# uzh-rpg/RVT

Hardware: AMD Instinct MI355X
Metric: event-tensors/sec (fwd+bwd) RVT-Base T=21 1Mpx; % MFMA roofline (higher is better)
Workload: dtype bf16; 1 GPU; RVT-Base, 1Mpx 20x360x640 (padded 384x640), T=21, B=24/GPU; global_batch=24, seq_len=21, parallelism=dp1, optimizer=AdamW(fused), hipgraph=off, upstream_grads=random cotangents on stage 2-4 features of all T frames

## Files before the change

### rvt_amd/csrc/attn_block.hpp

```cpp
#pragma once
#include "common.hpp"
#include "attn_pieces.hpp"
#include "opm.hpp"
#include "acc_frags.hpp"
#include "ln_pieces.hpp"

namespace rvt {

template <class T, int C> struct AbSmem {
    static constexpr int KT = C / TileGeom<T>::BK;
    static constexpr int W_QKV = KT * 3 * C * 128;
    static constexpr int W_P = KT * C * 128;
    static constexpr int OFF_P = W_QKV, OFF_K = W_QKV + W_P;
    static constexpr int K_LNW = 0, K_LNB = C, K_BQKV = 2 * C, K_BP = 5 * C, K_GAM = 6 * C, NCONST = 7 * C;
    static constexpr int OFF_S = OFF_K + NCONST * 4;
};

template <class T, int C>
__device__ __forceinline__ void ab_proj_t(f32x16& acc, const char* Wl, int wrows, int row0, const frag_t<T> (&uf)[C / 16], int li, int half) {
#pragma unroll
    for (int ks = 0; ks < C / 16; ks++) mma32(acc, opm_load_frag<T>(Wl, wrows, row0 + li, 2 * ks + half), uf[ks]);
}
template <class T, int C>
__device__ __forceinline__ void ab_proj_n(f32x16& acc, const char* Wl, int wrows, int row0, const frag_t<T> (&uf)[C / 16], int li, int half) {
// ... 358 lines not shown
#pragma unroll
            for (int bj = 0; bj < NB; bj++) {
                emit_dqkv(dk[bj], bj, r0 + 32);
                emit_dqkv(dv[bj], bj, r0 + 64);
            }
        }

#pragma unroll
        for (int b = 0; b < NB; b++) {
            float d8[KS][8];
#pragma unroll
            for (int cb = 0; cb < NCB; cb++) {
                float r8[2][8];
                acc_to_rows(du[cb][b], r8);
#pragma unroll
                for (int m = 0; m < 2; m++)
#pragma unroll
                    for (int e = 0; e < 8; e++) d8[2 * cb + m][e] = pt.valid[b] ? r8[m][e] : 0.f;
            }
            if (LN || PRE) {
                float gsum = 0.f, gxsum = 0.f;
                float xh[KS][8];
                if (PRE) {
#pragma unroll
                    for (int ks = 0; ks < KS; ks++)
#pragma unroll
                        for (int e = 0; e < 8; e++) d8[ks][e] += (float)df[b][ks][e];
                }
#pragma unroll
                for (int ks = 0; ks < KS; ks++) {
                    float w[8];
                    load_cols<8>(kst + S::K_LNW, 16 * ks + 8 * half, w);
                    const frag_t<T> xr = STASH ? *reinterpret_cast<const frag_t<T>*>(stash + (b * KS + ks) * 1024)
                                               : frag_load<T>((PRE ? y0 : x) + (size_t)pt.tok[b] * C + (2 * ks + half) * 8);
#pragma unroll
                    for (int e = 0; e < 8; e++) {
                        xh[ks][e] = pt.valid[b] ? ((float)xr[e] - mean[b]) * rstd[b] : 0.f;
                        const float gw = d8[ks][e] * w[e];
                        gsum += gw;
                        gxsum += gw * xh[ks][e];
                    }
                }
#pragma unroll
                for (int cb = 0; cb < NCB; cb++) {
                    f32x16 tw, tb;
                    acc_zero(tw);
                    acc_zero(tb);
#pragma unroll
                    for (int m = 0; m < 2; m++) {
                        float pw[8];
#pragma unroll
                        for (int e = 0; e < 8; e++) pw[e] = d8[2 * cb + m][e] * xh[2 * cb + m][e];
                        mma32(tw, frag_from_float<T>(pw), idf[m]);
                        mma32(tb, frag_from_float<T>(d8[2 * cb + m]), idf[m]);
                    }
#pragma unroll
                    for (int r = 0; r < 16; r++) { aw[cb] += tw[r]; ab[cb] += tb[r]; }
                }
                gsum += __shfl_xor(gsum, 32);
                gxsum += __shfl_xor(gxsum, 32);
                const float m1 = gsum / (float)C, m2 = gxsum / (float)C;
#pragma unroll
                for (int ks = 0; ks < KS; ks++) {
                    float w[8], o[8];
                    load_cols<8>(kst + S::K_LNW, 16 * ks + 8 * half, w);
#pragma unroll
                    for (int e = 0; e < 8; e++)
                        o[e] = (PRE ? 0.f : (float)df[b][ks][e]) + rstd[b] * (d8[ks][e] * w[e] - m1 - xh[ks][e] * m2);
                    if (pt.valid[b]) frag_store<T>(dx + (size_t)pt.tok[b] * C + (2 * ks + half) * 8, frag_from_float<T>(o));
                }
            } else {
#pragma unroll
                for (int ks = 0; ks < KS; ks++) {
                    float o[8];
#pragma unroll
                    for (int e = 0; e < 8; e++) o[e] = (float)df[b][ks][e] + d8[ks][e];
                    if (pt.valid[b]) frag_store<T>(dx + (size_t)pt.tok[b] * C + (2 * ks + half) * 8, frag_from_float<T>(o));
                }
            }
        }
    }
    if (LN || PRE) {
        float* const red = reinterpret_cast<float*>(smem + S::OFF_S + WPB * (SC::BYTES + DLN));
#pragma unroll
        for (int cb = 0; cb < NCB; cb++) {
            const float a = aw[cb] + __shfl_xor(aw[cb], 32), b = ab[cb] + __shfl_xor(ab[cb], 32);
            if (half == 0) {
                red[wave * 2 * C + 32 * cb + li] = a;
                red[wave * 2 * C + C + 32 * cb + li] = b;
            }
        }
        __syncthreads();
        for (int v = tid; v < 2 * C; v += 64 * WPB) {
            float sum = 0.f;
            for (int w = 0; w < WPB; w++) sum += red[w * 2 * C + v];
            atomicAdd((v < C ? dln_w : dln_b) + (v % C), sum);
        }
    }
}

}
```

### rvt_amd/csrc/mlp_chain.hpp

```cpp
#pragma once
#include "common.hpp"
#include "opm.hpp"
#include "acc_frags.hpp"
#include "ln_pieces.hpp"
#include "gelu_lut.hpp"

namespace rvt {

template <class T, int C> struct McSmem {
    static constexpr int KT = C / TileGeom<T>::BK, HID = 4 * C;
    static constexpr int W_1 = KT * HID * 128;
    static constexpr int W_2 = (HID / TileGeom<T>::BK) * C * 128;
    static constexpr int K_LNW = 0, K_LNB = C, K_B2 = 2 * C, K_GAM = 3 * C, K_B1 = 4 * C, NCONST = 8 * C;
};

template <class T, int C, int WPB, int MINW>
__global__ void __launch_bounds__(64 * WPB, MINW)
mlpc_fwd_kernel(const T* __restrict__ xmid, T* __restrict__ xout, const float* __restrict__ ln_w, const float* __restrict__ ln_b,
                const T* __restrict__ W1, const float* __restrict__ b1, const T* __restrict__ W2, const float* __restrict__ b2,
                const float* __restrict__ gamma, int M, float eps) {
    typedef McSmem<T, C> S;
    constexpr int KS = C / 16, NCB = C / 32, HID = 4 * C, NJC = HID / 32;
    __shared__ __attribute__((aligned(16))) char smem[S::W_1 + S::W_2 + S::NCONST * 4 + GeluTab<T>::BYTES];
    char* const W1_l = smem;
// ... 343 lines not shown
        }
        bf16x4 o;
#pragma unroll
        for (int r = 0; r < 4; r++) o[r] = (T)(acc[r] + acc2[r]);
        *reinterpret_cast<bf16x4*>(PB + buf * (32 * MCW_PP) + (16 * tb + l15) * MCW_PP + (16 * cq + 4 * kg) * 2) = o;
    };
    auto lnbwd = [&](const Stage& st, int buf, int tile, int slot) {
        if (!DGRAD || tile < 0 || tile >= n_tiles) return;
        const int row = tile * 32 + srow;
        const bf16x4 xb = __builtin_bit_cast(bf16x4, st.x), db = __builtin_bit_cast(bf16x4, st.d);
        const bf16x4 gb = *reinterpret_cast<const bf16x4*>(PB + buf * (32 * MCW_PP) + srow * MCW_PP + spc * 8);
        const float mean = MR[((slot & 3) * 32 + srow) * 2], rstd = MR[((slot & 3) * 32 + srow) * 2 + 1];
        float x[4];
#pragma unroll
        for (int i = 0; i < 4; i++) x[i] = (float)xb[i] - mean;
        float gw[4], s1 = 0.f, s2x = 0.f;
#pragma unroll
        for (int i = 0; i < 4; i++) {
            const float g = (float)gb[i];
            x[i] *= rstd;
            gw[i] = g * lw[i];
            s1 += gw[i];
            s2x += gw[i] * x[i];
            aw[i] += g * x[i];
            ab[i] += g;
        }
        const float m1 = row16_sum(s1) * (1.0f / C), m2 = row16_sum(s2x) * (1.0f / C);
        bf16x4 o;
#pragma unroll
        for (int i = 0; i < 4; i++) o[i] = (T)((float)db[i] + rstd * (gw[i] - m1 - x[i] * m2));
        if (row < M) *reinterpret_cast<bf16x4*>(dxmid + (size_t)row * C + 4 * spc) = o;
    };
    const bool mfma_first = wave < 4;
    const int t0 = blockIdx.x, G = gridDim.x;
    Stage sa, sb, sla, slb;
    fetch(sa, t0);
    fetch(sb, t0 + G);
    __syncthreads();
    stash(sa, t0, 0, 0);
    fetch(sa, t0 + 2 * G);
    if (DGRAD) fetch(sla, -1);
    lds_barrier();
    int k = 0;
    int tile = t0;
    for (; tile < n_tiles; tile += 2 * G, k += 2) {
        if (mfma_first) compute(0);
        stash(sb, tile + G, 1, k + 1);
        fetch(sb, tile + 3 * G);
        if (DGRAD) fetch(slb, tile - G);
        if (!mfma_first) compute(0);
        duty(1, tile - G, k - 1);
        lnbwd(sla, 0, tile - 2 * G, k - 2);
        lds_barrier();
        if (mfma_first && tile + G < n_tiles) compute(1);
        stash(sa, tile + 2 * G, 0, k + 2);
        fetch(sa, tile + 4 * G);
        if (DGRAD) fetch(sla, tile);
        if (!mfma_first && tile + G < n_tiles) compute(1);
        duty(0, tile, k);
        lnbwd(slb, 1, tile - G, k - 1);
        lds_barrier();
    }
    if (DGRAD) {
        fetch(slb, tile - G);
        duty(1, tile - G, k - 1);
        lnbwd(sla, 0, tile - 2 * G, k - 2);
        lds_barrier();
        lnbwd(slb, 1, tile - G, k - 1);
    }
    const size_t nwg = gridDim.x, wg = blockIdx.x;
    float* const p_dw1 = ws + wg * (size_t)(HID * C);
    float* const p_s2 = ws + nwg * (size_t)(HID * C) + wg * (size_t)(C * HID);
    float* const p_db1 = ws + 2 * nwg * (size_t)(HID * C) + (wg * 2) * (size_t)HID;
    float* const p_cs2 = ws + 2 * nwg * (size_t)(HID * C) + 2 * nwg * (size_t)HID + wg * (size_t)C;
#pragma unroll
    for (int cb = 0; cb < NCB; cb++)
#pragma unroll
        for (int r = 0; r < 16; r++) {
            p_dw1[(size_t)(32 * wave + acc_row(r, lane)) * C + 32 * cb + li] = dw1[cb][r];
            p_s2[(size_t)(32 * cb + acc_row(r, lane)) * HID + 32 * wave + li] = s2[cb][r];
        }
    db1 += __shfl_xor(db1, 32);
    if (half == 0) {
        p_db1[32 * wave + li] = db1;
        p_db1[HID + 32 * wave + li] = 0.f;
    }
    float* const red = reinterpret_cast<float*>(smem);
    __syncthreads();
#pragma unroll
    for (int i = 0; i < 4; i++) red[srow * C + 4 * spc + i] = cs[i];
    __syncthreads();
    if (tid < C) {
        float s = 0.f;
        for (int r = 0; r < 32; r++) s += red[r * C + tid];
        p_cs2[tid] = s;
    }
    if (DGRAD) {
        __syncthreads();
#pragma unroll
        for (int i = 0; i < 4; i++) { red[srow * C + 4 * spc + i] = aw[i]; red[32 * C + srow * C + 4 * spc + i] = ab[i]; }
        __syncthreads();
        if (tid < 2 * C) {
            float s = 0.f;
            for (int r = 0; r < 32; r++) s += red[(tid / C) * 32 * C + r * C + (tid % C)];
            atomicAdd((tid < C ? dln_w : dln_b) + (tid % C), s);
        }
    }
}

}
```

### rvt_amd/csrc/mlp_stream.hpp

```cpp
#pragma once
#include "common.hpp"
#include "lds_dma.hpp"
#include "opm.hpp"
#include "acc_frags.hpp"
#include "ln_pieces.hpp"
#include "gelu_lut.hpp"

namespace rvt {

template <class T, int C, int HC_ = TileGeom<T>::BK> struct MsGeom {
    static constexpr int BK = TileGeom<T>::BK;
    static constexpr int HC = HC_;
    static constexpr int KT = C / BK;
    static constexpr int HID = 4 * C, NCH = HID / HC, JPC = HC / 32;
    static constexpr int W1C = KT * HC * 128;
    static constexpr int W2C = C * 128;
    static constexpr int STAGE = W1C + W2C;
    static constexpr int K_LNW = 0, K_LNB = C, K_B2 = 2 * C, K_GAM = 3 * C, K_B1 = 4 * C, NCONST = 8 * C;
};

__device__ __forceinline__ int ms_rowperm(int li) { return (li & ~12) | ((li & 4) << 1) | ((li & 8) >> 1); }

template <class T, int C, int WPB, int MINW, int ABL = 0>
__global__ void __launch_bounds__(64 * WPB, MINW)
// ... 151 lines not shown
#pragma unroll
                for (int e = 0; e < 8; e++) o[e] = rs[e] + gam[e] * (r8[m][e] + b2v[e]);
                orow[ks] = frag_from_float<T>(o);
            }
        }
        prow = row;
        pvalid = valid;
    }
    if (pvalid) {
        const int half = lane_ >> 5;
#pragma unroll
        for (int ks = 0; ks < KS; ks++) frag_store<T>(xout + (size_t)prow * C + (2 * ks + half) * 8, orow[ks]);
    }
}



template <class T> struct MsTrAddr {
    int lo[2], hi[2];
    __device__ __forceinline__ void init(int lane, const char* smem) {
        const int rl = 4 * (lane >> 5) + ((lane & 15) >> 2), cl = 16 * ((lane >> 4) & 1) + 4 * (lane & 3);
        const int byte = cl * (int)sizeof(T);
#ifdef RVT_EMU
        const int base = 0;
        (void)smem;
#else
        const int base = (int)(size_t)(__attribute__((address_space(3))) const char*)(smem);
#endif
        const int l = rl * 128 + ((((byte >> 4) & 7) ^ ms_swz(rl)) << 4) + (byte & 15);
        const int h = (rl + 8) * 128 + ((((byte >> 4) & 7) ^ ms_swz(rl + 8)) << 4) + (byte & 15);
        lo[0] = base + l; lo[1] = base + (l ^ 64);
        hi[0] = base + h; hi[1] = base + (h ^ 64);
    }
};
#ifndef RVT_EMU
__device__ __forceinline__ void ms_lgkm_wait() {
    asm volatile("s_waitcnt lgkmcnt(0)" ::: "memory");
    __builtin_amdgcn_sched_barrier(0);
}
#else
__device__ __forceinline__ void ms_lgkm_wait() {}
#endif
template <int IMG, int ROWS, int ROW0, int CB>
__device__ __forceinline__ bf16x8 ms_tr_frag(const char* smem, const MsTrAddr<bf16>& a) {
    constexpr int OFF = IMG + (CB / 2) * ROWS * 128 + ROW0 * 128;
#ifdef RVT_EMU
    return frag_from_tr<bf16>(reinterpret_cast<const bf16*>(smem + OFF + a.lo[CB & 1]), reinterpret_cast<const bf16*>(smem + OFF + a.hi[CB & 1]));
#else
    typedef __attribute__((ext_vector_type(2))) unsigned int u32x2_t;
    u32x2_t lo, hi2;
    asm volatile("ds_read_b64_tr_b16 %0, %1 offset:%2" : "=v"(lo) : "v"(a.lo[CB & 1]), "n"(OFF));
    asm volatile("ds_read_b64_tr_b16 %0, %1 offset:%2" : "=v"(hi2) : "v"(a.hi[CB & 1]), "n"(OFF));
    const u32x4 v = {lo[0], lo[1], hi2[0], hi2[1]};
    bf16x8 f;
    __builtin_memcpy(&f, &v, 16);
    return f;
#endif
}
template <int ROWS>
__device__ __forceinline__ f32x8 ms_tr_frag_f32(const char* img, int row0, int col0, int lane) {
    f32x8 f;
#pragma unroll
    for (int e = 0; e < 8; e++) {
        const int row = row0 + (e & 3) + 8 * (e >> 2) + 4 * (lane >> 5), col = col0 + (lane & 31);
        const int byte = (col % 32) * 4;
        f[e] = *reinterpret_cast<const float*>(img + (col / 32) * ROWS * 128 + row * 128 + ((((byte >> 4) & 7) ^ ms_swz(row)) << 4) + (byte & 15));
    }
    return f;
}

template <class T, int C, int WPB, int MINW>
__global__ void __launch_bounds__(64 * WPB, MINW)
mlps_bwd_dgrad_kernel(const T* __restrict__ dxout, const T* __restrict__ xmid, T* __restrict__ dxmid,
                      const float* __restrict__ ln_w, const float* __restrict__ ln_b, const T* __restrict__ W1,
                      const float* __restrict__ b1, const T* __restrict__ W2gT, float* __restrict__ dln_w,
                      float* __restrict__ dln_b, int M, float eps) {
    typedef MsGeom<T, C, 32> G;
    constexpr int KS = C / 16, NCB = C / 32, HID = 4 * C, NCH = G::NCH, JPC = G::JPC;
    constexpr int NPW = (G::W1C / 1024) / WPB;
    static_assert(NPW * WPB * 1024 == G::W1C, "chunk pieces must divide over the waves");
    constexpr int STAGE = 2 * G::W1C;
    constexpr int DT = G::KT * 32 * 128;
    constexpr int OFF_DT = 2 * STAGE, OFF_K = OFF_DT + WPB * DT, OFF_LUT = OFF_K + G::NCONST * 4, OFF_PF = OFF_LUT + GeluTab<T>::BYTES;
    __shared__ __attribute__((aligned(16))) char smem[OFF_PF + 1024];
    float* const kst = reinterpret_cast<float*>(smem + OFF_K);
    float* const lut = reinterpret_cast<float*>(smem + OFF_LUT);
    const int tid = threadIdx.x, lane_ = tid & 63;
    const int wave = wave_uniform(tid >> 6);
    GeluTab<T>::template fill<true>(lut, tid, 64 * WPB);
    for (int i = tid; i < C; i += 64 * WPB) { kst[G::K_LNW + i] = ln_w[i]; kst[G::K_LNB + i] = ln_b[i]; }
    for (int i = tid; i < HID; i += 64 * WPB) kst[G::K_B1 + i] = b1[i];
    __syncthreads();

    const pp_rsrc r1 = pp_make_rsrc(W1, (unsigned)(HID * C * sizeof(T))), r2 = pp_make_rsrc(W2gT, (unsigned)(HID * C * sizeof(T)));
    auto issue = [&](int ch, int stage) __attribute__((always_inline)) {
        int lane = lane_;
        opaque_vgpr(lane);
        int v[NPW];
        ms_piece_offsets<T, NPW, WPB>(v, wave, lane, G::HC, C);
#pragma unroll
        for (int i = 0; i < NPW; i++) {
            const int p = wave + i * WPB;
            pp_glds16(r1, smem, stage * STAGE + p * 1024, v[i], ch * (G::HC * C * (int)sizeof(T)));
            pp_glds16(r2, smem, stage * STAGE + G::W1C + p * 1024, v[i], ch * (G::HC * C * (int)sizeof(T)));
        }
    };

    float aw[NCB], ab[NCB];
#pragma unroll
    for (int cb = 0; cb < NCB; cb++) { aw[cb] = 0.f; ab[cb] = 0.f; }

    const int n_tiles = (M + 31) / 32;
    const int n_wg = (n_tiles + WPB - 1) / WPB;
    char* const pf_dummy = smem + OFF_PF;
    issue(0, 0);
    frag_t<T> orow[KS];
    int prow = 0;
    bool pvalid = false;
    for (int twg = blockIdx.x; twg < n_wg; twg += gridDim.x) {
        int lane = lane_;
        opaque_vgpr(lane);
        const int li = lane & 31, half = lane >> 5;
        const int rb = ms_rowbase_h<T>(li, half);
        const int rbd = OFF_DT + wave * DT + rb;
        MsTrAddr<T> ta;
        ta.init(lane, smem);
        const int tile = twg * WPB + wave;
        const int row = tile * 32 + li;
        const bool valid = tile < n_tiles && row < M;
        const bool more = twg + (int)gridDim.x < n_wg;
        frag_t<T> uf[KS];
        float mean, rstd;
        {
            frag_t<T> xf[KS], df[KS];
            mc_load_row<T, C>(xf, xmid, row, valid, half);
            mc_load_row<T, C>(df, dxout, row, valid, half);
#pragma unroll
            for (int ks = 0; ks < KS; ks++) ms_store_frag<T>(smem, 32, rbd, 2 * ks, df[ks]);
            mc_layernorm<T, C>(xf, uf, kst + G::K_LNW, kst + G::K_LNB, valid, half, eps, mean, rstd);
        }
        f32x16 dacc[NCB];
#pragma unroll
        for (int cb = 0; cb < NCB; cb++) acc_zero(dacc[cb]);
        auto boundary = [&](int ch, int stage_next) __attribute__((always_inline)) {
            pp_wait_vm<0>();
            pp_barrier();
            if (ch + 1 < NCH) issue(ch + 1, stage_next);
            else if (more) issue(0, stage_next);
        };
        auto compute = [&](int ch, auto stage_c) __attribute__((always_inline)) {
            constexpr int STG = decltype(stage_c)::value;
            const char* const W1s = smem + STG * STAGE;
            const char* const W2s = W1s + G::W1C;
#pragma unroll
            for (int jj = 0; jj < JPC; jj++) {
                f32x16 h, dg;
                acc_load_rows(h, kst + G::K_B1 + ch * G::HC + 32 * jj, half);
                acc_zero(dg);
#pragma unroll
                for (int ks = 0; ks < KS; ks++) {
                    mma32(h, ms_load_frag<T>(W1s + 32 * jj * 128, G::HC, rb, 2 * ks), uf[ks]);
                    mma32(dg, ms_load_frag<T>(W2s + 32 * jj * 128, G::HC, rb, 2 * ks), ms_load_frag<T>(smem, 32, rbd, 2 * ks));
                }
                sched_fence();
                frag_t<T> wt[NCB][2];
                static_for<JPC>([&](auto jj_c) {
                    if (decltype(jj_c)::value != jj) return;
                    static_for<NCB * 2>([&](auto i_c) {
                        constexpr int JJ = decltype(jj_c)::value, CB = decltype(i_c)::value / 2, Q = decltype(i_c)::value % 2;
                        if constexpr (sizeof(T) == 2) wt[CB][Q] = ms_tr_frag<STG * STAGE, G::HC, 32 * JJ + 16 * Q, CB>(smem, ta);
                        else wt[CB][Q] = ms_tr_frag_f32<G::HC>(W1s, 32 * JJ + 16 * Q, CB * 32, lane);
                    });
                });
                float dh[16];
                GeluTab<T>::eval16(lut, h, dh);
#pragma unroll
                for (int r = 0; r < 16; r++) dh[r] = mul_nopack(dh[r], dg[r], r);
                frag_t<T> dhf[2];
                dhf[0] = arr_slot_frag<T>(dh, 0);
                dhf[1] = arr_slot_frag<T>(dh, 1);
                if constexpr (sizeof(T) == 2) ms_lgkm_wait();
#pragma unroll
                for (int cb = 0; cb < NCB; cb++)
#pragma unroll
                    for (int q = 0; q < 2; q++) mma32(dacc[cb], wt[cb][q], dhf[q]);
            }
        };
        boundary(0, 1);
        if (pvalid) {
#pragma unroll
            for (int ks = 0; ks < KS; ks++) frag_store<T>(dxmid + (size_t)prow * C + (2 * ks + half) * 8, orow[ks]);
        }
        compute(0, std::integral_constant<int, 0>());
#pragma unroll 1
        for (int ch = 1; ch < NCH - 1; ch += 2) {
            boundary(ch, 0);
            if (ch == 1 && more) {
                const int tn = tile + (int)gridDim.x * WPB;
                if (tn < n_tiles) {
                    const int rows = M - tn * 32 < 32 ? M - tn * 32 : 32;
                    const pp_rsrc rx = pp_make_rsrc(xmid + (size_t)tn * 32 * C, (unsigned)(rows * C * sizeof(T)));
                    const pp_rsrc rd = pp_make_rsrc(dxout + (size_t)tn * 32 * C, (unsigned)(rows * C * sizeof(T)));
#pragma unroll
                    for (int i = 0; i < (32 * C * (int)sizeof(T)) / 1024; i++) {
                        pp_glds16(rx, smem, (int)(pf_dummy - smem), lane * 16 + i * 1024, 0);
                        pp_glds16(rd, smem, (int)(pf_dummy - smem), lane * 16 + i * 1024, 0);
                    }
                }
            }
            compute(ch, std::integral_constant<int, 1>());
            boundary(ch + 1, 1);
            compute(ch + 1, std::integral_constant<int, 0>());
        }
        boundary(NCH - 1, 0);
        compute(NCH - 1, std::integral_constant<int, 1>());
        sched_fence();
        frag_t<T> xf[KS];
#pragma unroll
        for (int ks = 0; ks < KS; ks++) xf[ks] = frag_load<T>(xmid + (size_t)(valid ? row : 0) * C + (2 * ks + half) * 8);
        frag_t<T> idf[2];
#pragma unroll
        for (int m = 0; m < 2; m++)
#pragma unroll
            for (int e = 0; e < 8; e++) idf[m][e] = (T)((16 * m + 8 * half + e == li) ? 1.0f : 0.0f);
        float gsum = 0.f, gxsum = 0.f;
#pragma unroll
        for (int cb = 0; cb < NCB; cb++) {
            float r8[2][8];
            acc_to_rows(dacc[cb], r8);
            f32x16 tw, tb;
            acc_zero(tw);
            acc_zero(tb);
#pragma unroll
            for (int m = 0; m < 2; m++) {
                const int ks = 2 * cb + m;
                float w[8], pw[8], d[8];
                load_cols<8>(kst + G::K_LNW, 16 * ks + 8 * half, w);
#pragma unroll
                for (int e = 0; e < 8; e++) {
                    d[e] = valid ? r8[m][e] : 0.f;
                    const float xh = valid ? ((float)xf[ks][e] - mean) * rstd : 0.f;
                    const float gw = d[e] * w[e];
                    gsum += gw;
                    gxsum += gw * xh;
                    pw[e] = d[e] * xh;
                }
                mma32(tw, frag_from_float<T>(pw), idf[m]);
                mma32(tb, frag_from_float<T>(d), idf[m]);
            }
#pragma unroll
            for (int r = 0; r < 16; r++) { aw[cb] += tw[r]; ab[cb] += tb[r]; }
        }
        gsum += __shfl_xor(gsum, 32);
        gxsum += __shfl_xor(gxsum, 32);
        const float m1 = gsum / (float)C, m2 = gxsum / (float)C;
#pragma unroll
        for (int cb = 0; cb < NCB; cb++) {
            float r8[2][8];
#ifndef RVT_EMU
            asm volatile("" : "+v"(dacc[cb]));
#endif
            acc_to_rows(dacc[cb], r8);
#pragma unroll
            for (int m = 0; m < 2; m++) {
                const int ks = 2 * cb + m;
                float w[8], o[8];
                load_cols<8>(kst + G::K_LNW, 16 * ks + 8 * half, w);
                const frag_t<T> dfk = ms_load_frag<T>(smem, 32, rbd, 2 * ks);
#pragma unroll
                for (int e = 0; e < 8; e++) {
                    const float xh = ((float)xf[ks][e] - mean) * rstd;
                    o[e] = (float)dfk[e] + rstd * (r8[m][e] * w[e] - m1 - xh * m2);
                }
                orow[ks] = frag_from_float<T>(o);
            }
        }
        prow = row;
        pvalid = valid;
    }
    const int li = lane_ & 31, half = lane_ >> 5;
    if (pvalid) {
#pragma unroll
        for (int ks = 0; ks < KS; ks++) frag_store<T>(dxmid + (size_t)prow * C + (2 * ks + half) * 8, orow[ks]);
    }
    pp_wait_vm<0>();
    __syncthreads();
    float* const red = reinterpret_cast<float*>(smem);
#pragma unroll
    for (int cb = 0; cb < NCB; cb++) {
        const float a = aw[cb] + __shfl_xor(aw[cb], 32), b = ab[cb] + __shfl_xor(ab[cb], 32);
        if (half == 0) {
            red[wave * 2 * C + 32 * cb + li] = a;
            red[wave * 2 * C + C + 32 * cb + li] = b;
        }
    }
    __syncthreads();
    for (int v = tid; v < 2 * C; v += 64 * WPB) {
        float sum = 0.f;
        for (int w = 0; w < WPB; w++) sum += red[w * 2 * C + v];
        atomicAdd((v < C ? dln_w : dln_b) + (v % C), sum);
    }
}

struct MswGeom {
    static constexpr int C = 128, HID = 512, HB = 256, KS = 8, NCB = 4;
    static constexpr int TILE = 32 * 256;
    static constexpr int W2P = 272, W2IMG = HB * W2P;
    static constexpr int OFF_XV = 0, OFF_DX = 3 * TILE, OFF_W2 = 6 * TILE, OFF_LUT = OFF_W2 + W2IMG, OFF_K = OFF_LUT + GELU_NLUT_BYTES;
    static constexpr int SMEM = OFF_K + 2 * C * 4;
};
__device__ __forceinline__ int msw_tile_off(int row, int chunk) { return row * 256 + ((chunk ^ (row & 15)) << 4); }

template <int TAG>
__global__ void __launch_bounds__(512, 2)
mlps_bwd_wgrad_kernel(const bf16* __restrict__ dxout, const bf16* __restrict__ xmid, const float* __restrict__ ln_w,
                      const float* __restrict__ ln_b, const bf16* __restrict__ W1, const float* __restrict__ b1,
                      const bf16* __restrict__ W2gT, float* __restrict__ ws, int M, float eps, int nstreams) {
    typedef bf16 T;
    typedef MswGeom G;
    constexpr int C = G::C, KS = G::KS, NCB = G::NCB, HID = G::HID, TILE = G::TILE;
    __shared__ __attribute__((aligned(16))) char smem[G::SMEM];
    float* const lut = reinterpret_cast<float*>(smem + G::OFF_LUT);
    float* const kst = reinterpret_cast<float*>(smem + G::OFF_K);
    const int tid = threadIdx.x, lane_ = tid & 63;
    const int wave = wave_uniform(tid >> 6);
    const int bid = blockIdx.x;
    const int hb = (bid >> 3) & 1, stream = (bid >> 4) * 8 + (bid & 7);
    if (stream >= nstreams) return;
    const int n_tiles = (M + 31) / 32;
    const int count = stream < n_tiles ? (n_tiles - stream + nstreams - 1) / nstreams : 0;

    gelu_nlut_fill<false>(lut, tid, 512);
    for (int i = tid; i < C; i += 512) { kst[i] = ln_w[i]; kst[C + i] = ln_b[i]; }
    for (int f = tid; f < G::HB * 16; f += 512) {
        const int r = f >> 4, c = f & 15;
        *reinterpret_cast<u32x4*>(smem + G::OFF_W2 + r * G::W2P + c * 16) =
            *reinterpret_cast<const u32x4*>(W2gT + (size_t)(hb * G::HB + r) * C + c * 8);
    }
    const int jrow = hb * G::HB + 32 * wave + (lane_ & 31);
    frag_t<T> w1f[KS];
#pragma unroll
    for (int ks = 0; ks < KS; ks++) w1f[ks] = frag_load<T>(W1 + (size_t)jrow * C + 16 * ks + 8 * (lane_ >> 5));
    const float b1v = b1[jrow];

    f32x16 dw1[NCB], s2[NCB];
#pragma unroll
    for (int cb = 0; cb < NCB; cb++) { acc_zero(dw1[cb]); acc_zero(s2[cb]); }
    float db1 = 0.f;
    float cs1 = 0.f;
    const int cs_cb = wave & 3, cs_q = wave >> 2;

    auto issue = [&](int k, int buf) __attribute__((always_inline)) {
        int lane = lane_;
        opaque_vgpr(lane);
        const int tile = stream + k * nstreams;
        const int rows = tile < n_tiles ? (M - tile * 32 < 32 ? M - tile * 32 : 32) : 0;
        const pp_rsrc rx = pp_make_rsrc(xmid + (size_t)(rows ? tile : 0) * 32 * C, (unsigned)(rows * C * 2));
        const pp_rsrc rd = pp_make_rsrc(dxout + (size_t)(rows ? tile : 0) * 32 * C, (unsigned)(rows * C * 2));
        const int r = 4 * wave + (lane >> 4), c = (lane & 15) ^ (r & 15);
        const int voff = r * 256 + c * 16;
        pp_glds16(rx, smem, G::OFF_XV + buf * TILE + wave * 1024, voff, 0);
        pp_glds16(rd, smem, G::OFF_DX + buf * TILE + wave * 1024, voff, 0);
    };
    auto layernorm = [&](int buf, bool live) __attribute__((always_inline)) {
        if (!live) return;
        int t = tid;
        opaque_vgpr(t);
        const int srow = t >> 4, spc = t & 15;
        char* const px = smem + G::OFF_XV + buf * TILE + msw_tile_off(srow, spc);
        const bf16x8 xb = *reinterpret_cast<const bf16x8*>(px);
        float x[8], s = 0.f;
#pragma unroll
        for (int i = 0; i < 8; i++) { x[i] = (float)xb[i]; s += x[i]; }
// ... 149 lines not shown
```

### rvt_amd/csrc/ppgemm.hpp

```cpp
#pragma once
#include <type_traits>
#include "common.hpp"
#include "lds_dma.hpp"

namespace rvt {

struct PPMat {
    const bf16* p0; const bf16* p1; int ld; int kcut;
};

enum { PP_STORE = 0,
       PP_SCALE_RES = 1,
       PP_GELU_DUAL = 2,
       PP_MUL = 3,
       PP_ADD = 4 };
struct PPEpArgs {
    bf16* out; bf16* out2; const bf16* side; const float* c0; const float* c1; int ld;
};

struct PPGeom {
    static constexpr int BM = 256, BN = 256, BK = 64;
    static constexpr int UNIT = 64 * 128;
    static constexpr int STAGE = 8 * UNIT;
    static constexpr int OFF_W = 4 * UNIT;
// ... 120 lines not shown
            if (++lkt == nk_of(nt)) { lkt = 0; lu++; }
        } else {
            d.rx = pp_make_rsrc(X.p0, 0u); d.rw = pp_make_rsrc(W.p0, 0u); d.sx = 0; d.sw = 0;
        }
        lstep++;
        return d;
    };
    auto issue_x = [&](const Desc& d, int stage, int i) __attribute__((always_inline)) {
        int v = vx0 + i * ldx64;
        if (GATHER == 2) {
            const int m = d.mask + (lr >> 5) * 128 + i * 32 + (lr & 31);
            uint32_t f, rem, oy, ox;
            cv.dHoWo.divmod((uint32_t)(m < M ? m : 0), f, rem);
            cv.dWo.divmod(rem, oy, ox);
            const int pix = ((int)f * cv.H + 2 * (int)oy - 1 + d.da) * cv.W + 2 * (int)ox - 1 + d.db;
            const bool kill = m >= M || ((int)oy == 0 && d.da == 0) || ((int)ox == 0 && d.db == 0);
            v = kill ? (int)0x80000000u : pix * cv.Cout * 2 + chunk * 16;
        } else if (GATHER) {
            const bool kill = ((d.mask >> i) & 1) | (d.da & (d.mask >> (4 + i)) & 1) | (d.db & (d.mask >> (8 + i)) & 1);
            v = kill ? (int)0x80000000u : v;
        }
        if (!(ABL & 1)) pp_glds16(d.rx, smem, stage * G::STAGE + i * G::UNIT + lds0, v, d.sx);
    };
    auto issue_w = [&](const Desc& d, int stage, int g) __attribute__((always_inline)) {
        if (!(ABL & 1)) pp_glds16(d.rw, smem, stage * G::STAGE + G::OFF_W + g * G::UNIT + lds0, vw0 + g * ldw128, d.sw);
    };

    f32x16 acc[4][2];
    bf16x8 xf[4], wf[2][4];

    struct OutDesc { pp_rsrc out, out2, side; int n0, m0; };
    auto out_desc = [&](int mt, int nt) -> OutDesc {
        OutDesc o;
        const int rows = M - mt * G::BM;
        const unsigned bytes = GATHER == 1 ? (unsigned)((size_t)(M / (cv.Ho * cv.Wo)) * cv.H * cv.W * cv.Cin * 2)
                                           : (unsigned)((rows > G::BM ? G::BM : rows) * ep.ld * 2);
        const size_t base = GATHER == 1 ? 0 : (size_t)mt * G::BM * ep.ld;
        o.m0 = mt * G::BM;
        o.out = pp_make_rsrc(ep.out + base, (ABL & 32) ? 0u : bytes);
        o.out2 = pp_make_rsrc(ep.out2 ? ep.out2 + base : ep.out, ep.out2 ? bytes : 0u);
        o.side = pp_make_rsrc(ep.side ? ep.side + base : ep.out, ep.side ? bytes : 0u);
        o.n0 = nt * G::BN;
        return o;
    };
    char* const scr = smem + G::OFF_SCR + wc * G::SCR_BYTES;
    auto row_voff = [&](int i, int it, const OutDesc& od, int lane) __attribute__((always_inline)) {
        const int r = wr * 128 + i * 32 + it * 8 + (lane >> 3), pc = lane & 7, colb = od.n0 + wc * 64;
        int voff = (r * ep.ld + colb + 8 * pc) * 2;
        if (GATHER == 1) {
            const int m = od.m0 + r;
            uint32_t f, rem, a, b;
            cv.dHoWo.divmod((uint32_t)(m < M ? m : 0), f, rem);
            cv.dWo.divmod(rem, a, b);
            const int cls = colb / cv.Cin, cb = colb - cls * cv.Cin;
            const int pix = ((int)f * cv.H + 2 * (int)a + (cls >> 1)) * cv.W + 2 * (int)b + (cls & 1);
            voff = m < M ? (pix * cv.Cin + cb + 8 * pc) * 2 : (int)0xfffffff0u;
        }
        return voff;
    };
    auto side_load = [&](int i, const OutDesc& od, u32x4 (&sd)[4]) __attribute__((always_inline)) {
        if (!SIDE || (ABL & 16)) return;
        int lane = lane_;
#ifndef RVT_EMU
        asm volatile("" : "+v"(lane));
#endif
#pragma unroll
        for (int it = 0; it < 4; it++) sd[it] = pp_load16(od.side, row_voff(i, it, od, lane));
    };
    auto flush_block = [&](int i, const OutDesc& od, const u32x4 (&sd)[4]) __attribute__((always_inline)) {
        if (ABL & 16) {
#ifndef RVT_EMU
            asm volatile("" ::"v"(acc[i][0]), "v"(acc[i][1]));
#endif
            return;
        }
        int lane = lane_, l31, hi;
#ifndef RVT_EMU
        asm volatile("" : "+v"(lane));
#endif
        l31 = lane & 31; hi = lane >> 5;
        const int row0 = wr * 128 + i * 32;
        const int colb = od.n0 + wc * 64;
        typedef __attribute__((ext_vector_type(4))) __bf16 bf16x4;
        auto convert = [&](int j, bool second) __attribute__((always_inline)) {
            float v[16];
#pragma unroll
            for (int g = 0; g < 4; g++) {
                const int n = colb + 32 * j + 8 * g + 4 * hi;
                const f32x4 c0 = *reinterpret_cast<const f32x4*>(cst + n);
#pragma unroll
                for (int w = 0; w < 4; w++) v[4 * g + w] = acc[i][j][4 * g + w] + c0[w];
                if (EP == PP_SCALE_RES) {
                    const f32x4 c1 = *reinterpret_cast<const f32x4*>(cst + c1off + n);
#pragma unroll
                    for (int w = 0; w < 4; w++) v[4 * g + w] *= c1[w];
                }
            }
            if (EP == PP_GELU_DUAL) {
#pragma unroll
                for (int h8 = 0; h8 < 2; h8++) {
                    float x8[8], g8[8], p8[8];
#pragma unroll
                    for (int e = 0; e < 8; e++) x8[e] = v[8 * h8 + e];
                    gelu_both_8(x8, g8, p8);
#pragma unroll
                    for (int e = 0; e < 8; e++) v[8 * h8 + e] = second ? p8[e] : g8[e];
                }
            }
#pragma unroll
            for (int g = 0; g < 4; g++) {
                bf16x4 t;
#pragma unroll
                for (int w = 0; w < 4; w++) t[w] = (bf16)v[4 * g + w];
                *reinterpret_cast<bf16x4*>(scr + l31 * G::SCR_LD + (32 * j + 8 * g + 4 * hi) * 2) = t;
            }
        };
        auto store_rows = [&](const pp_rsrc& dst, bool apply_side) __attribute__((always_inline)) {
#pragma unroll
            for (int it = 0; it < 4; it++) {
                const int r = it * 8 + (lane >> 3), pc = lane & 7;
                const int voff = row_voff(i, it, od, lane);
                u32x4 t = *reinterpret_cast<const u32x4*>(scr + r * G::SCR_LD + pc * 16);
                if (SIDE && apply_side) {
                    bf16x8 a, b;
                    __builtin_memcpy(&a, &t, 16);
                    __builtin_memcpy(&b, &sd[it], 16);
                    float o[8];
#pragma unroll
                    for (int e = 0; e < 8; e++) o[e] = EP == PP_MUL ? (float)a[e] * (float)b[e] : (float)a[e] + (float)b[e];
                    const bf16x8 rv = frag_from_float<bf16>(o);
                    __builtin_memcpy(&t, &rv, 16);
                }
                pp_store16(dst, voff, t);
            }
        };
        convert(0, false);
        convert(1, false);
        pp_wave_sync();
        store_rows(od.out, true);
        if (EP == PP_GELU_DUAL) {
            pp_wave_sync();
            convert(0, true);
            convert(1, true);
            pp_wave_sync();
            store_rows(od.out2, false);
        }
        pp_wave_sync();
    };

    __syncthreads();
    Desc d1, d2;
    {
        const Desc d0 = next_desc();
#pragma unroll
        for (int g = 0; g < 4; g++) issue_w(d0, 0, g);
#pragma unroll
        for (int i = 0; i < 4; i++) issue_x(d0, 0, i);
        d1 = next_desc();
#pragma unroll
        for (int g = 0; g < 4; g++) issue_w(d1, 1, g);
        d2 = next_desc();
    }
    if (!(ABL & 1)) pp_wait_vm<7>();
    pp_barrier();
    if (wr == 1) pp_barrier();

    int s = 0;
    OutDesc od = out_desc(0, 0);
    auto bar = [&]() { if (!(ABL & 8)) pp_barrier(); };
    auto xfrag = [&](int st, int i, int ks) __attribute__((always_inline)) {
        if (ABL & 2) { bf16x8 v; for (int e = 0; e < 8; e++) v[e] = (bf16)(float)(st + i + ks + lane); return v; }
        return *reinterpret_cast<const bf16x8*>(smem + ((st + xaddr0) ^ (ks << 5)) + i * G::UNIT);
    };
    auto wfrag = [&](int st, int j, int ks) __attribute__((always_inline)) {
        if (ABL & 2) { bf16x8 v; for (int e = 0; e < 8; e++) v[e] = (bf16)(float)(st + j + ks - lane); return v; }
        return *reinterpret_cast<const bf16x8*>(smem + ((st + waddr0) ^ (ks << 5)) + j * 4096);
    };
    auto step_body = [&](auto mode_c) __attribute__((always_inline)) {
        constexpr int MODE = decltype(mode_c)::value;
        constexpr bool FIRST = MODE == 1 || MODE == 3, FLUSH = MODE == 1;
        constexpr int ST = (ABL & 16) ? 0 : (EP == PP_GELU_DUAL ? 8 : 4) + ((ABL & 64) ? 4 : 0);
        constexpr int SL = (SIDE && !(ABL & 16)) ? 4 : 0;
        constexpr bool PREF = GATHER != 1;
        constexpr int E0 = ST + (PREF ? 2 * SL : SL), E1 = ST + SL, E2 = ST + SL, E3 = ST + (PREF ? 0 : SL);
        constexpr int W0 = 8 + (MODE == 2 ? E0 + E1 + E2 + E3 : 0), W1 = 9 + (MODE == 1 ? E0 : MODE == 2 ? E1 + E2 + E3 : 0),
                      W2 = 10 + (MODE == 1 ? E0 + E1 : MODE == 2 ? E1 + E2 + E3 : 0), W3 = 7 + (MODE == 1 ? E0 + E1 + E2 : 0);
        u32x4 sda[4], sdb[4];
        int st = (s & 1) * G::STAGE;
#ifndef RVT_EMU
        asm volatile("" : "+v"(st));
#endif
        auto mfmas = [&](int i) __attribute__((always_inline)) {
            pp_setprio(1);
#pragma unroll
            for (int ks = 0; ks < 4; ks++) {
                if (ABL & 4) { if (FIRST && ks == 0) { acc_zero(acc[i][0]); acc_zero(acc[i][1]); } acc[i][0][ks] += (float)wf[0][ks][0] * (float)xf[ks][1]; continue; }
                if (FIRST && ks == 0) { mma32_zero(acc[i][0], wf[0][ks], xf[ks]); mma32_zero(acc[i][1], wf[1][ks], xf[ks]); }
                else { mma32(acc[i][0], wf[0][ks], xf[ks]); mma32(acc[i][1], wf[1][ks], xf[ks]); }
            }
            pp_setprio(0);
        };
        issue_x(d1, (s + 1) & 1, 0); issue_x(d1, (s + 1) & 1, 1);
        if (!(ABL & 1)) pp_wait_vm<W0>();
        if (FLUSH) { side_load(0, od, sda); if (PREF) side_load(1, od, sdb); flush_block(0, od, sda); }
#pragma unroll
        for (int ks = 0; ks < 4; ks++) { wf[0][ks] = wfrag(st, 0, ks); xf[ks] = xfrag(st, 0, ks); wf[1][ks] = wfrag(st, 1, ks); }
        bar();
        mfmas(0);
        bar();
        issue_x(d1, (s + 1) & 1, 2); issue_x(d1, (s + 1) & 1, 3);
        if (!(ABL & 1)) pp_wait_vm<W1>();
        if (FLUSH) { if (PREF) { side_load(2, od, sda); flush_block(1, od, sdb); } else { side_load(1, od, sda); flush_block(1, od, sda); } }
#pragma unroll
        for (int ks = 0; ks < 4; ks++) xf[ks] = xfrag(st, 1, ks);
        bar();
        mfmas(1);
        bar();
        issue_w(d2, s & 1, 0); issue_w(d2, s & 1, 1);
        if (!(ABL & 1)) pp_wait_vm<W2>();
        if (FLUSH) { if (PREF) { side_load(3, od, sdb); flush_block(2, od, sda); } else { side_load(2, od, sda); flush_block(2, od, sda); } }
#pragma unroll
        for (int ks = 0; ks < 4; ks++) xf[ks] = xfrag(st, 2, ks);
        bar();
        mfmas(2);
        bar();
        issue_w(d2, s & 1, 2); issue_w(d2, s & 1, 3);
// ... 58 lines not shown
```

Before: 7663 event-tensors/s.

## Park GELU derivative in registers and move LN-grad accumulators to LDS

Result: no change. 7714 event-tensors/s (median of 6 runs) (+0.7%).

```diff
diff --git a/profiles/microbench_gelu_dual.py b/profiles/microbench_gelu_dual.py
--- /dev/null
+++ b/profiles/microbench_gelu_dual.py
@@ -0,0 +1,43 @@
+import os, sys, torch
+sys.path.insert(0, os.path.dirname(os.path.dirname(os.path.abspath(__file__))))
+from rvt_amd import ops, tuning
+
+dev, dt = torch.device('cuda', 0), torch.bfloat16
+
+
+def timeit(fn, n=15):
+    for _ in range(3):
+        fn()
+    torch.cuda.synchronize()
+    ts = []
+    for _ in range(n):
+        e0, e1 = torch.cuda.Event(enable_timing=True), torch.cuda.Event(enable_timing=True)
+        e0.record(); fn(); e1.record(); torch.cuda.synchronize()
+        ts.append(e0.elapsed_time(e1))
+    ts.sort()
+    return ts[n // 2], ts[0], ts[-1]
+
+
+def rnd(*shape, scale=1.0):
+    return (torch.randn(*shape, device=dev) * scale).to(dt)
+
+
+lib = os.environ.get('RVT_HIP_LIB', 'tree')
+for M, N, K in [(120960, 2048, 512), (483840, 1024, 256)]:
+    x, w, b = rnd(M, K), rnd(N, K, scale=0.05), torch.randn(N, device=dev)
+    if K == 512:
+        t = timeit(lambda: ops.linear_gelu_fwd(x, w, b, want_grad=True))
+        print(f'[{lib}] ({M},{N},{K}) gelu dual, 256-wide engine: median {t[0]:.4f} min {t[1]:.4f} max {t[2]:.4f} ms', flush=True)
+        t = timeit(lambda: ops.linear_gelu_fwd(x, w, b, want_grad=False))
+        print(f'[{lib}] ({M},{N},{K}) gelu only (gp = NULL), 256-wide engine: median {t[0]:.4f} min {t[1]:.4f} max {t[2]:.4f} ms', flush=True)
+        mul, y = rnd(M, N), torch.empty(M, N, device=dev, dtype=dt)
+        t = timeit(lambda: ops.linear_dgrad(x, w, mul=mul, out=y))
+        print(f'[{lib}] ({M},{N},{K}) PP_MUL: median {t[0]:.4f} min {t[1]:.4f} max {t[2]:.4f} ms', flush=True)
+        del mul, y
+    else:
+        t = timeit(lambda: ops.linear_gelu_fwd(x, w, b, want_grad=True))
+        print(f'[{lib}] ({M},{N},{K}) gelu dual, lin_gelu_ws_kernel (route in use): median {t[0]:.4f} min {t[1]:.4f} max {t[2]:.4f} ms', flush=True)
+        with tuning.override(ln_linear=0, ppgemm_all=1):
+            t = timeit(lambda: ops.linear_gelu_fwd(x, w, b, want_grad=True))
+        print(f'[{lib}] ({M},{N},{K}) gelu dual, 256-wide engine (ln_linear=0, ppgemm_all=1): median {t[0]:.4f} min {t[1]:.4f} max {t[2]:.4f} ms', flush=True)
+    del x, w, b
diff --git a/rvt_amd/csrc/attn_block.hpp b/rvt_amd/csrc/attn_block.hpp
--- a/rvt_amd/csrc/attn_block.hpp
+++ b/rvt_amd/csrc/attn_block.hpp
@@ -464,12 +464,15 @@
     }
     if (LN || PRE) {
         float* const red = reinterpret_cast<float*>(smem + S::OFF_S + WPB * (SC::BYTES + DLN));
+        int t = tid;
+        opaque_vgpr(t);
+        const int slot = (t >> 6) * 2 * C + (t & 31);
 #pragma unroll
         for (int cb = 0; cb < NCB; cb++) {
             const float a = aw[cb] + __shfl_xor(aw[cb], 32), b = ab[cb] + __shfl_xor(ab[cb], 32);
             if (half == 0) {
-                red[wave * 2 * C + 32 * cb + li] = a;
-                red[wave * 2 * C + C + 32 * cb + li] = b;
+                red[slot + 32 * cb] = a;
+                red[slot + C + 32 * cb] = b;
             }
         }
         __syncthreads();
diff --git a/rvt_amd/csrc/mlp_chain.hpp b/rvt_amd/csrc/mlp_chain.hpp
--- a/rvt_amd/csrc/mlp_chain.hpp
+++ b/rvt_amd/csrc/mlp_chain.hpp
@@ -449,8 +449,11 @@
         }
     db1 += __shfl_xor(db1, 32);
     if (half == 0) {
-        p_db1[32 * wave + li] = db1;
-        p_db1[HID + 32 * wave + li] = 0.f;
+        int t = tid;
+        opaque_vgpr(t);
+        const int j = 32 * (t >> 6) + (t & 31);
+        p_db1[j] = db1;
+        p_db1[HID + j] = 0.f;
     }
     float* const red = reinterpret_cast<float*>(smem);
     __syncthreads();
diff --git a/rvt_amd/csrc/mlp_stream.hpp b/rvt_amd/csrc/mlp_stream.hpp
--- a/rvt_amd/csrc/mlp_stream.hpp
+++ b/rvt_amd/csrc/mlp_stream.hpp
@@ -257,7 +257,8 @@
     constexpr int STAGE = 2 * G::W1C;
     constexpr int DT = G::KT * 32 * 128;
     constexpr int OFF_DT = 2 * STAGE, OFF_K = OFF_DT + WPB * DT, OFF_LUT = OFF_K + G::NCONST * 4, OFF_PF = OFF_LUT + GeluTab<T>::BYTES;
-    __shared__ __attribute__((aligned(16))) char smem[OFF_PF + 1024];
+    constexpr int OFF_LNG = OFF_PF + 1024, LNG = 2 * NCB * 64 * 4;
+    __shared__ __attribute__((aligned(16))) char smem[OFF_LNG + WPB * LNG];
     float* const kst = reinterpret_cast<float*>(smem + OFF_K);
     float* const lut = reinterpret_cast<float*>(smem + OFF_LUT);
     const int tid = threadIdx.x, lane_ = tid & 63;
@@ -281,17 +282,18 @@
         }
     };
 
-    float aw[NCB], ab[NCB];
-#pragma unroll
-    for (int cb = 0; cb < NCB; cb++) { aw[cb] = 0.f; ab[cb] = 0.f; }
+    float* const lng = reinterpret_cast<float*>(smem + OFF_LNG + wave * LNG);
+#pragma unroll
+    for (int k = 0; k < 2 * NCB; k++) lng[k * 64 + lane_] = 0.f;
 
     const int n_tiles = (M + 31) / 32;
     const int n_wg = (n_tiles + WPB - 1) / WPB;
     char* const pf_dummy = smem + OFF_PF;
     issue(0, 0);
     frag_t<T> orow[KS];
-    int prow = 0;
+    int ptwg = 0;
     bool pvalid = false;
+    auto prow_of = [&](int lane) __attribute__((always_inline)) { return (ptwg * WPB + wave) * 32 + (lane & 31); };
     for (int twg = blockIdx.x; twg < n_wg; twg += gridDim.x) {
         int lane = lane_;
         opaque_vgpr(lane);
@@ -363,6 +365,7 @@
         };
         boundary(0, 1);
         if (pvalid) {
+            const int prow = prow_of(lane);
 #pragma unroll
             for (int ks = 0; ks < KS; ks++) frag_store<T>(dxmid + (size_t)prow * C + (2 * ks + half) * 8, orow[ks]);
         }
@@ -423,8 +426,11 @@
                 mma32(tw, frag_from_float<T>(pw), idf[m]);
                 mma32(tb, frag_from_float<T>(d), idf[m]);
             }
-#pragma unroll
-            for (int r = 0; r < 16; r++) { aw[cb] += tw[r]; ab[cb] += tb[r]; }
+            float aw = lng[cb * 64 + lane], ab = lng[(NCB + cb) * 64 + lane];
+#pragma unroll
+            for (int r = 0; r < 16; r++) { aw += tw[r]; ab += tb[r]; }
+            lng[cb * 64 + lane] = aw;
+            lng[(NCB + cb) * 64 + lane] = ab;
         }
         gsum += __shfl_xor(gsum, 32);
         gxsum += __shfl_xor(gxsum, 32);
@@ -450,20 +456,24 @@
                 orow[ks] = frag_from_float<T>(o);
             }
         }
-        prow = row;
+        ptwg = twg;
         pvalid = valid;
     }
     const int li = lane_ & 31, half = lane_ >> 5;
     if (pvalid) {
+        const int prow = prow_of(lane_);
 #pragma unroll
         for (int ks = 0; ks < KS; ks++) frag_store<T>(dxmid + (size_t)prow * C + (2 * ks + half) * 8, orow[ks]);
     }
     pp_wait_vm<0>();
     __syncthreads();
     float* const red = reinterpret_cast<float*>(smem);
+    int lane = lane_;
+    opaque_vgpr(lane);
 #pragma unroll
     for (int cb = 0; cb < NCB; cb++) {
-        const float a = aw[cb] + __shfl_xor(aw[cb], 32), b = ab[cb] + __shfl_xor(ab[cb], 32);
+        const float aw = lng[cb * 64 + lane], ab = lng[(NCB + cb) * 64 + lane];
+        const float a = aw + __shfl_xor(aw, 32), b = ab + __shfl_xor(ab, 32);
         if (half == 0) {
             red[wave * 2 * C + 32 * cb + li] = a;
             red[wave * 2 * C + C + 32 * cb + li] = b;
diff --git a/rvt_amd/csrc/ppgemm.hpp b/rvt_amd/csrc/ppgemm.hpp
--- a/rvt_amd/csrc/ppgemm.hpp
+++ b/rvt_amd/csrc/ppgemm.hpp
@@ -226,7 +226,8 @@
         const int row0 = wr * 128 + i * 32;
         const int colb = od.n0 + wc * 64;
         typedef __attribute__((ext_vector_type(4))) __bf16 bf16x4;
-        auto convert = [&](int j, bool second) __attribute__((always_inline)) {
+        bf16x4 gpk[2][4];
+        auto convert = [&](int j) __attribute__((always_inline)) {
             float v[16];
 #pragma unroll
             for (int g = 0; g < 4; g++) {
@@ -248,7 +249,12 @@
                     for (int e = 0; e < 8; e++) x8[e] = v[8 * h8 + e];
                     gelu_both_8(x8, g8, p8);
 #pragma unroll
-                    for (int e = 0; e < 8; e++) v[8 * h8 + e] = second ? p8[e] : g8[e];
+                    for (int e = 0; e < 8; e++) v[8 * h8 + e] = g8[e];
+#pragma unroll
+                    for (int e = 0; e < 8; e++) gpk[j][2 * h8 + (e >> 2)][e & 3] = (bf16)p8[e];
+#ifndef RVT_EMU
+                    asm volatile("" : "+v"(gpk[j][2 * h8]), "+v"(gpk[j][2 * h8 + 1]));
+#endif
                 }
             }
 #pragma unroll
@@ -258,6 +264,11 @@
                 for (int w = 0; w < 4; w++) t[w] = (bf16)v[4 * g + w];
                 *reinterpret_cast<bf16x4*>(scr + l31 * G::SCR_LD + (32 * j + 8 * g + 4 * hi) * 2) = t;
             }
+        };
+        auto unpark = [&](int j) __attribute__((always_inline)) {
+#pragma unroll
+            for (int g = 0; g < 4; g++)
+                *reinterpret_cast<bf16x4*>(scr + l31 * G::SCR_LD + (32 * j + 8 * g + 4 * hi) * 2) = gpk[j][g];
         };
         auto store_rows = [&](const pp_rsrc& dst, bool apply_side) __attribute__((always_inline)) {
 #pragma unroll
@@ -278,14 +289,14 @@
                 pp_store16(dst, voff, t);
             }
         };
-        convert(0, false);
-        convert(1, false);
+        convert(0);
+        convert(1);
         pp_wave_sync();
         store_rows(od.out, true);
         if (EP == PP_GELU_DUAL) {
             pp_wave_sync();
-            convert(0, true);
-            convert(1, true);
+            unpark(0);
+            unpark(1);
             pp_wave_sync();
             store_rows(od.out2, false);
         }
```
